# MayDomine/Burst-Attention

Measured on NVIDIA H100. Metric: attention fwd+bwd TFLOPS/s (bs=1, H=32, d=128, bf16; seq in config, default 262144 on N > 1 GPUs, 65536 on one), aggregate over GPUs, higher is better.
Workload: dtype bf16

## Files before the change

### burst-attention_b200/csrc/fwd_sm90.cuh

```cuda
#pragma once
#include <math.h>
#include <stdlib.h>

#include "doc_sm90.cuh"
#include "host_common.h"
#include "sm90_ptx.cuh"

namespace ba {

constexpr int kBlockM = 128;
constexpr int kBlockN = 128;
constexpr int kKStages = 2;
constexpr int kVStages = 2;
constexpr int kBoxBytes = 128 * 64 * 2;
constexpr int kFwdThreads = 384;

struct FwdParams {
  float* o_acc;
  int64_t oacc_sb, oacc_ss, oacc_sh;
  float* lse;
  int64_t lse_sb, lse_sh;
  void* o_out;
  int64_t oout_sb, oout_ss, oout_sh;
  int B, Sq, Sk, H;
  int G;
  float scale_log2;
  const float* bias;
  int64_t bias_sb, bias_sh;
  int causal;
  int causal_off;
  int load_state;
  int store_lowp;
  int lo;
  const float* slopes;
  int64_t slopes_sb;
  int64_t dist0;
  int pstride;
  const int* cu;
  int n_docs;
  int q_pos0, k_pos0;
};

struct __align__(8) FwdBarriers {
  uint64_t q_full;
  uint64_t k_full[kKStages], k_empty[kKStages];
  uint64_t b_full[kKStages];
  uint64_t v_full[kVStages], v_empty[kVStages];
};

template <int kD>
struct FwdLayout {
  static_assert(kD == 64 || kD == 128, "head dim 64 or 128");
  static constexpr uint32_t kTileB = 128 * kD * 2;
  static constexpr int kBoxes = kD / 64;
  static constexpr uint32_t kOffQ = 0;
  static constexpr uint32_t kOffK = kTileB;
  static constexpr uint32_t kOffV = kOffK + kKStages * kTileB;
  static constexpr uint32_t kOffBias = kOffV + kVStages * kTileB;
  static constexpr uint32_t kOffBars = kOffBias + kKStages * kBlockN * 4;
  static constexpr int kSmemBytes = kOffBars + 256 ;
  static_assert(kSmemBytes <= 232448, "forward kernel exceeds 227 KiB of shared memory");
};

__device__ __forceinline__ int fwd_trip_count(int r0, const FwdParams& p) {
  if (r0 >= p.Sq) return 0;
  int r_last = min(r0 + 63, p.Sq - 1);
  int max_limit = p.causal ? min(r_last + p.causal_off, p.Sk - 1) : p.Sk - 1;
  return max_limit < 0 ? 0 : max_limit / kBlockN + 1;
}

__device__ __forceinline__ int fwd_first_tile(int r0, const FwdParams& p) { return max(0, r0 + p.lo) / kBlockN; }

__device__ __forceinline__ void fwd_doc_range(int r0, const FwdParams& p, int* first, int* end) {
  *first = *end = 0;
  if (r0 >= p.Sq) return;
  const int r_last = min(r0 + 63, p.Sq - 1);
  int k_lo, k_hi, unused;
  doc_interval(p.q_pos0 + p.pstride * r0, p.cu, p.n_docs, p.k_pos0, p.pstride, p.Sk, &k_lo, &unused);
  doc_interval(p.q_pos0 + p.pstride * r_last, p.cu, p.n_docs, p.k_pos0, p.pstride, p.Sk, &unused, &k_hi);
  const int f = max(fwd_first_tile(r0, p), k_lo / kBlockN);
  const int e = min(fwd_trip_count(r0, p), (k_hi + kBlockN - 1) / kBlockN);
  if (e > f) *first = f, *end = e;
}

__device__ __forceinline__ int64_t alibi_dref(int a, const FwdParams& p) {
  const int64_t hi = (int64_t)p.pstride * a + p.dist0, lo = hi - (int64_t)p.pstride * (p.Sk - 1);
  return max((int64_t)0, max(lo, -hi));
}

__device__ __forceinline__ int64_t alibi_carried_ref(int64_t dref, float m0, float slope2) {
  if (slope2 > 0.f) {
    const float cap = fmaxf(0.f, -m0) / slope2;
    if (cap < (float)dref) return (int64_t)cap;
  }
  return dref;
}

template <bool kBF16, int kD, bool kBias, bool kBand, bool kAlibi, bool kDoc = false>
__device__ __forceinline__ void fwd_chunk_body(const CUtensorMap& tmQ, const CUtensorMap& tmK, const CUtensorMap& tmV,
                                               const FwdParams& p) {
  static_assert(!(kBias && kAlibi), "ALiBi is not combined with the key bias");
  static_assert(!kDoc || (kBand && !kBias && !kAlibi), "documents run on the band path, without key bias or ALiBi");
  extern __shared__ __align__(1024) uint8_t smem_raw[];
  uint8_t* smem = smem_raw;
  if ((smem_u32(smem) & 1023u) != 0) __trap();
  using L = FwdLayout<kD>;
  constexpr uint32_t kTileBytes = L::kTileB;
  constexpr int kBoxes = L::kBoxes, kOReg = kD / 2;
  uint8_t* sQ = smem + L::kOffQ;
  uint8_t* sK = smem + L::kOffK;
  uint8_t* sV = smem + L::kOffV;
  float* sBias = reinterpret_cast<float*>(smem + L::kOffBias);
  FwdBarriers* bars = reinterpret_cast<FwdBarriers*>(smem + L::kOffBars);

  const int warp = __shfl_sync(0xffffffffu, threadIdx.x >> 5, 0);
  const int lane = threadIdx.x & 31;
  const int h = blockIdx.y, b = blockIdx.z;
  const int row0 = (p.causal ? (int)(gridDim.x - 1 - blockIdx.x) : (int)blockIdx.x) * kBlockM;
  int n_tiles = max(fwd_trip_count(row0, p), fwd_trip_count(row0 + 64, p));
  int t0 = 0;
  if constexpr (kBand) {
    t0 = min(fwd_first_tile(row0, p), n_tiles);
    n_tiles -= t0;
  }
  if constexpr (kDoc) {
    int f0, e0, f1, e1;
    fwd_doc_range(row0, p, &f0, &e0);
    fwd_doc_range(row0 + 64, p, &f1, &e1);
    t0 = e0 > f0 ? (e1 > f1 ? min(f0, f1) : f0) : f1;
    n_tiles = max(0, max(e0, e1) - t0);
  }

  if (threadIdx.x == 0) {
    tma_prefetch_desc(&tmQ);
    tma_prefetch_desc(&tmK);
    tma_prefetch_desc(&tmV);
    mbar_init(&bars->q_full, 1);
    for (int i = 0; i < kKStages; ++i) {
      mbar_init(&bars->k_full[i], 1);
      mbar_init(&bars->k_empty[i], 8);
      mbar_init(&bars->b_full[i], 1);
    }
    for (int i = 0; i < kVStages; ++i) {
      mbar_init(&bars->v_full[i], 1);
      mbar_init(&bars->v_empty[i], 8);
    }
    fence_mbar_init();
  }
  __syncthreads();

  if (warp < 4) {
    reg_alloc_dec<40>();
    if (warp != 0) return;
    const int hk = h / p.G;
    if (lane == 0) {
      mbar_arrive_expect_tx(&bars->q_full, kTileBytes);
      for (int half = 0; half < kBoxes; ++half)
        tma_load_4d(sQ + half * kBoxBytes, &tmQ, &bars->q_full, half * 64, h, row0, b);
    }
    for (int i = 0; i < n_tiles; ++i) {
      const int ks = i % kKStages, kph = (i / kKStages) & 1;
      mbar_wait(&bars->k_empty[ks], kph ^ 1);
      if (lane == 0) {
        mbar_arrive_expect_tx(&bars->k_full[ks], kTileBytes);
        for (int half = 0; half < kBoxes; ++half)
          tma_load_4d(sK + ks * kTileBytes + half * kBoxBytes, &tmK, &bars->k_full[ks], half * 64, hk,
                      (t0 + i) * kBlockN, b);
      }
      if constexpr (kBias) {
#pragma unroll
        for (int j = 0; j < 4; ++j) {
          const int key = (t0 + i) * kBlockN + lane + 32 * j;
          float x = 0.f;
          if (key < p.Sk) x = __ldg(p.bias + (int64_t)b * p.bias_sb + (int64_t)h * p.bias_sh + key) * kLog2e;
          sBias[ks * kBlockN + lane + 32 * j] = x;
        }
        __syncwarp();
        if (lane == 0) mbar_arrive(&bars->b_full[ks]);
      }
      if (lane == 0) {
        const int vs = i % kVStages, vph = (i / kVStages) & 1;
        mbar_wait(&bars->v_empty[vs], vph ^ 1);
        mbar_arrive_expect_tx(&bars->v_full[vs], kTileBytes);
        for (int half = 0; half < kBoxes; ++half)
          tma_load_4d(sV + vs * kTileBytes + half * kBoxBytes, &tmV, &bars->v_full[vs], half * 64, hk,
                      (t0 + i) * kBlockN, b);
      }
      __syncwarp();
    }
    return;
  }

  reg_alloc_inc<232>();
  const int wg = (threadIdx.x >> 7) - 1;
  const int w = warp & 3, g = lane >> 2, t = lane & 3;
  const int r_lo = row0 + wg * 64 + 16 * w + g;
  const int rows[2] = {r_lo, r_lo + 8};
  [[maybe_unused]] int doc_first = 0, doc_end = 0, doc_lo[2] = {0, 0}, doc_hi[2] = {0, 0};
  if constexpr (kDoc) {
    fwd_doc_range(row0 + wg * 64, p, &doc_first, &doc_end);
#pragma unroll
    for (int r = 0; r < 2; ++r)
      if (rows[r] < p.Sq)
        doc_interval(p.q_pos0 + p.pstride * rows[r], p.cu, p.n_docs, p.k_pos0, p.pstride, p.Sk, &doc_lo[r], &doc_hi[r]);
  }
  const int n_mine = kDoc ? doc_end : fwd_trip_count(row0 + wg * 64, p);
  const float scale_log2 = p.scale_log2;
  int limit[2];
#pragma unroll
  for (int r = 0; r < 2; ++r) limit[r] = p.causal ? min(rows[r] + p.causal_off, p.Sk - 1) : p.Sk - 1;
  if constexpr (kDoc) {
#pragma unroll
    for (int r = 0; r < 2; ++r) limit[r] = min(limit[r], doc_hi[r] - 1);
  }
  const int limit_min = min(limit[0], limit[1]);
  int my0 = 0, lo_limit[2] = {0, 0};
  if constexpr (kBand) {
    my0 = fwd_first_tile(row0 + wg * 64, p);
    lo_limit[0] = rows[0] + p.lo;
    lo_limit[1] = rows[1] + p.lo;
  }
  if constexpr (kDoc) {
    my0 = doc_first;
#pragma unroll
    for (int r = 0; r < 2; ++r) lo_limit[r] = max(lo_limit[r], doc_lo[r]);
  }
  const int lo_limit_max = max(lo_limit[0], lo_limit[1]);
  float slope2 = 0.f;
  int64_t dref[2] = {0, 0};
  if constexpr (kAlibi) {
    slope2 = __ldg(p.slopes + (int64_t)b * p.slopes_sb + h) * kLog2e;
    dref[0] = alibi_dref(rows[0], p);
    dref[1] = alibi_dref(rows[1], p);
  }

  float o[kOReg];
  float m[2] = {-INFINITY, -INFINITY}, l[2] = {0.f, 0.f};
#pragma unroll
  for (int i = 0; i < kOReg; ++i) o[i] = 0.f;
  if (p.load_state) {
#pragma unroll
    for (int r = 0; r < 2; ++r) {
      if (rows[r] >= p.Sq) continue;
      const float lse_prev = p.lse[(int64_t)b * p.lse_sb + (int64_t)h * p.lse_sh + rows[r]];
      if (lse_prev != -INFINITY) {
        m[r] = lse_prev * kLog2e;
        if constexpr (kAlibi) {
          dref[r] = alibi_carried_ref(dref[r], m[r], slope2);
          m[r] += slope2 * (float)dref[r];
        }
        l[r] = t == 0 ? 1.f : 0.f;
      }
      const float* src = p.o_acc + (int64_t)b * p.oacc_sb + (int64_t)rows[r] * p.oacc_ss + (int64_t)h * p.oacc_sh;
#pragma unroll
      for (int c = 0; c < kD / 8; ++c) {
        const float2 f = __ldg(reinterpret_cast<const float2*>(src + 8 * c + 2 * t));
        o[4 * c + 2 * r] = f.x;
        o[4 * c + 2 * r + 1] = f.y;
      }
    }
  }

  const uint32_t q_base = smem_u32(sQ) + wg * 64 * 128;
  mbar_wait(&bars->q_full, 0);
  for (int i = 0; i < n_tiles; ++i) {
    const int ks = i % kKStages, kph = (i / kKStages) & 1;
    const int vs = i % kVStages, vph = (i / kVStages) & 1;
    const bool work = kBand ? (t0 + i >= my0 && t0 + i < n_mine) : i < n_mine;
    mbar_wait(&bars->k_full[ks], kph);
    float sc[64];
    if (work) {
      const uint32_t k_base = smem_u32(sK + ks * kTileBytes);
      wgmma_fence();
#pragma unroll
      for (int kk = 0; kk < kD / 16; ++kk) {
        const uint32_t off = (kk >> 2) * kBoxBytes + (kk & 3) * 32;
        wgmma_ss_n128<kBF16, 0, 0>(sc, make_desc(q_base + off, 16, 1024), make_desc(k_base + off, 16, 1024),
                                   kk > 0 ? 1u : 0u);
      }
      wgmma_commit();
      wgmma_wait<0>();
      fence_regs<64>(sc);
      const int key0 = (t0 + i) * kBlockN;
      if constexpr (kBias) {
        mbar_wait(&bars->b_full[ks], kph);
        const float* bias = sBias + ks * kBlockN;
#pragma unroll
        for (int c = 0; c < 16; ++c) {
          const float2 bb = *reinterpret_cast<const float2*>(bias + 8 * c + 2 * t);
#pragma unroll
          for (int r = 0; r < 2; ++r) {
            sc[4 * c + 2 * r] = fmaf(sc[4 * c + 2 * r], scale_log2, bb.x);
            sc[4 * c + 2 * r + 1] = fmaf(sc[4 * c + 2 * r + 1], scale_log2, bb.y);
          }
        }
      } else if constexpr (kAlibi) {
        const int64_t base = (int64_t)p.pstride * (row0 + wg * 64 - key0) + p.dist0;
        const int64_t dmin = base - (int64_t)p.pstride * (kBlockN - 1), dmax = base + (int64_t)p.pstride * 63;
        const float pf = (float)p.pstride;
        if (dmin >= 0 || dmax <= 0) {
          const int sg = dmin >= 0 ? 1 : -1;
          float rowb[2];
#pragma unroll
          for (int r = 0; r < 2; ++r)
            rowb[r] = -slope2 * (float)(sg * ((int64_t)p.pstride * (rows[r] - key0) + p.dist0) - dref[r]);
          const float ks = sg > 0 ? slope2 * pf : -slope2 * pf, kt = ks * (float)(2 * t);
#pragma unroll
          for (int c = 0; c < 16; ++c)
#pragma unroll
            for (int e = 0; e < 4; ++e)
              sc[4 * c + e] = fmaf(sc[4 * c + e], scale_log2, rowb[e >> 1] + fmaf(ks, (float)(8 * c + (e & 1)), kt));
        } else {
          float dr[2], dreff[2];
#pragma unroll
          for (int r = 0; r < 2; ++r) {
            dr[r] = (float)((int64_t)p.pstride * (rows[r] - key0 - 2 * t) + p.dist0);
            dreff[r] = slope2 * (float)dref[r];
          }
#pragma unroll
          for (int c = 0; c < 16; ++c)
#pragma unroll
            for (int e = 0; e < 4; ++e)
              sc[4 * c + e] = fmaf(-slope2, fabsf(fmaf(-pf, (float)(8 * c + (e & 1)), dr[e >> 1])),
                                   fmaf(sc[4 * c + e], scale_log2, dreff[e >> 1]));
        }
      } else {
#pragma unroll
        for (int j = 0; j < 64; ++j) sc[j] *= scale_log2;
      }
      if (key0 + kBlockN - 1 > limit_min) {
#pragma unroll
        for (int c = 0; c < 16; ++c)
#pragma unroll
          for (int e = 0; e < 4; ++e)
            if (key0 + 8 * c + 2 * t + (e & 1) > limit[e >> 1]) sc[4 * c + e] = -INFINITY;
      }
      if constexpr (kBand) {
        if (key0 < lo_limit_max) {
#pragma unroll
          for (int c = 0; c < 16; ++c)
#pragma unroll
            for (int e = 0; e < 4; ++e)
              if (key0 + 8 * c + 2 * t + (e & 1) < lo_limit[e >> 1]) sc[4 * c + e] = -INFINITY;
        }
      }
    }
    __syncwarp();
    if (lane == 0) mbar_arrive(&bars->k_empty[ks]);
    if (work) {
      uint32_t pa[32];
#pragma unroll
      for (int r = 0; r < 2; ++r) {
        float mx = -INFINITY;
#pragma unroll
        for (int c = 0; c < 16; ++c) mx = fmaxf(mx, fmaxf(sc[4 * c + 2 * r], sc[4 * c + 2 * r + 1]));
        mx = fmaxf(mx, __shfl_xor_sync(0xffffffffu, mx, 1));
        mx = fmaxf(mx, __shfl_xor_sync(0xffffffffu, mx, 2));
        const float m_new = fmaxf(m[r], mx);
        const float f = (m[r] == -INFINITY) ? 0.f : ex2(m[r] - m_new);
        const float neg_m = (m_new == -INFINITY) ? 0.f : -m_new;
        m[r] = m_new;
        float sum = 0.f;
#pragma unroll
        for (int c = 0; c < 16; ++c) {
          const float p0 = ex2(sc[4 * c + 2 * r] + neg_m), p1 = ex2(sc[4 * c + 2 * r + 1] + neg_m);
          sc[4 * c + 2 * r] = p0;
          sc[4 * c + 2 * r + 1] = p1;
          sum += p0 + p1;
        }
        l[r] = l[r] * f + sum;
#pragma unroll
        for (int c = 0; c < kD / 8; ++c) {
          o[4 * c + 2 * r] *= f;
          o[4 * c + 2 * r + 1] *= f;
        }
      }
#pragma unroll
      for (int j = 0; j < 32; ++j) pa[j] = pack2<kBF16>(sc[2 * j], sc[2 * j + 1]);
      mbar_wait(&bars->v_full[vs], vph);
      const uint32_t v_base = smem_u32(sV + vs * kTileBytes);
      fence_regs<32>(pa);
      fence_regs<kOReg>(o);
      wgmma_fence();
#pragma unroll
      for (int kk = 0; kk < kBlockN / 16; ++kk) {
        const uint64_t dv = make_desc(v_base + kk * 16 * 128, kBoxBytes, 1024);
        if constexpr (kD == 128) wgmma_rs_n128<kBF16, 1>(o, pa + 4 * kk, dv, 1u);
        else wgmma_rs_n64<kBF16, 1>(o, pa + 4 * kk, dv, 1u);
      }
      wgmma_commit();
      wgmma_wait<0>();
      fence_regs<kOReg>(o);
    } else {
      mbar_wait(&bars->v_full[vs], vph);
    }
    __syncwarp();
    if (lane == 0) mbar_arrive(&bars->v_empty[vs]);
  }

#pragma unroll
  for (int r = 0; r < 2; ++r) {
    float lr = l[r];
    lr += __shfl_xor_sync(0xffffffffu, lr, 1);
    lr += __shfl_xor_sync(0xffffffffu, lr, 2);
    const int row = rows[r];
    if (row >= p.Sq) continue;
    const float inv_l = lr > 0.f ? 1.f / lr : 0.f;
    if constexpr (kAlibi) {
      if (t == 0)
        p.lse[(int64_t)b * p.lse_sb + (int64_t)h * p.lse_sh + row] =
            lr > 0.f ? (m[r] + lg2(lr) - slope2 * (float)dref[r]) * kLn2 : -INFINITY;
    } else {
      if (t == 0) p.lse[(int64_t)b * p.lse_sb + (int64_t)h * p.lse_sh + row] = lr > 0.f ? (m[r] + lg2(lr)) * kLn2 : -INFINITY;
    }
    if (p.store_lowp) {
      uint16_t* dst = reinterpret_cast<uint16_t*>(p.o_out) + (int64_t)b * p.oout_sb + (int64_t)row * p.oout_ss +
                      (int64_t)h * p.oout_sh + 2 * t;
#pragma unroll
      for (int c = 0; c < kD / 8; ++c)
        *reinterpret_cast<uint32_t*>(dst + 8 * c) = pack2<kBF16>(o[4 * c + 2 * r] * inv_l, o[4 * c + 2 * r + 1] * inv_l);
    } else {
      float* dst = p.o_acc + (int64_t)b * p.oacc_sb + (int64_t)row * p.oacc_ss + (int64_t)h * p.oacc_sh + 2 * t;
#pragma unroll
      for (int c = 0; c < kD / 8; ++c)
        *reinterpret_cast<float2*>(dst + 8 * c) = make_float2(o[4 * c + 2 * r] * inv_l, o[4 * c + 2 * r + 1] * inv_l);
    }
  }
}

template <bool kBF16, int kD, bool kBias, bool kBand>
__global__ void __launch_bounds__(kFwdThreads, 1)
fwd_chunk_kernel(const __grid_constant__ CUtensorMap tmQ, const __grid_constant__ CUtensorMap tmK,
                 const __grid_constant__ CUtensorMap tmV, const FwdParams p) {
  fwd_chunk_body<kBF16, kD, kBias, kBand, false>(tmQ, tmK, tmV, p);
}

template <bool kBF16, int kD, bool kBand>
__global__ void __launch_bounds__(kFwdThreads, 1)
fwd_alibi_kernel(const __grid_constant__ CUtensorMap tmQ, const __grid_constant__ CUtensorMap tmK,
                 const __grid_constant__ CUtensorMap tmV, const FwdParams p) {
  fwd_chunk_body<kBF16, kD, false, kBand, true>(tmQ, tmK, tmV, p);
}

template <bool kBF16, int kD>
__global__ void __launch_bounds__(kFwdThreads, 1)
fwd_doc_kernel(const __grid_constant__ CUtensorMap tmQ, const __grid_constant__ CUtensorMap tmK,
               const __grid_constant__ CUtensorMap tmV, const FwdParams p) {
  fwd_chunk_body<kBF16, kD, false, true, false, true>(tmQ, tmK, tmV, p);
}

template <bool kBand>
inline int launch_fwd(int dtype, int D, bool bias, const CUtensorMap& tmQ, const CUtensorMap& tmK,
                      const CUtensorMap& tmV, const FwdParams& p, cudaStream_t stream) {
  const bool bf16 = dtype == BA_DTYPE_BF16;
  void (*kern)(CUtensorMap, CUtensorMap, CUtensorMap, FwdParams);
  if (bias)
    kern = D == 64 ? (bf16 ? fwd_chunk_kernel<true, 64, true, kBand> : fwd_chunk_kernel<false, 64, true, kBand>)
                   : (bf16 ? fwd_chunk_kernel<true, 128, true, kBand> : fwd_chunk_kernel<false, 128, true, kBand>);
  else
    kern = D == 64 ? (bf16 ? fwd_chunk_kernel<true, 64, false, kBand> : fwd_chunk_kernel<false, 64, false, kBand>)
                   : (bf16 ? fwd_chunk_kernel<true, 128, false, kBand> : fwd_chunk_kernel<false, 128, false, kBand>);
  const int smem = D == 64 ? FwdLayout<64>::kSmemBytes : FwdLayout<128>::kSmemBytes;
  BA_CHECK_CUDA(cudaFuncSetAttribute(kern, cudaFuncAttributeMaxDynamicSharedMemorySize, smem));
  dim3 grid((p.Sq + kBlockM - 1) / kBlockM, p.H, p.B);
  kern<<<grid, kFwdThreads, smem, stream>>>(tmQ, tmK, tmV, p);
  BA_CHECK_CUDA(cudaGetLastError());
  return BA_OK;
}

int launch_fwd_band(int dtype, int D, bool bias, const CUtensorMap& tmQ, const CUtensorMap& tmK,
                    const CUtensorMap& tmV, const FwdParams& p, cudaStream_t stream);
int launch_fwd_alibi(int dtype, int D, bool band, const CUtensorMap& tmQ, const CUtensorMap& tmK,
                     const CUtensorMap& tmV, const FwdParams& p, cudaStream_t stream);
int launch_fwd_doc(int dtype, int D, const CUtensorMap& tmQ, const CUtensorMap& tmK, const CUtensorMap& tmV,
                   const FwdParams& p, cudaStream_t stream);

}
```

Before: 503.2.

## Overlap QK^T of next tile with PV of previous tile in forward consumer

Restructures the consumer warpgroup loop into a software pipeline. The S=QK^T wgmma for tile i is issued together with the P·V wgmma for tile i-1, so softmax of tile i runs while the PV matmul is in flight. Skipped tiles outside the work range are now handled by separate pre and post loops that only cycle the barriers. This costs extra live registers, since sc, pa and o are all held at once, which risks spills and also changes the K/V release ordering.

```diff
diff --git a/burst-attention_b200/csrc/fwd_sm90.cuh b/burst-attention_b200/csrc/fwd_sm90.cuh
--- a/burst-attention_b200/csrc/fwd_sm90.cuh
+++ b/burst-attention_b200/csrc/fwd_sm90.cuh
@@ -262,141 +262,187 @@
   }
 
   const uint32_t q_base = smem_u32(sQ) + wg * 64 * 128;
+  int s_begin = 0, s_end = n_mine;
+  if constexpr (kBand) s_begin = max(my0 - t0, 0), s_end = n_mine - t0;
+  s_begin = min(s_begin, n_tiles);
+  s_end = max(min(s_end, n_tiles), s_begin);
+
+  const auto wait_k = [&](int i) { mbar_wait(&bars->k_full[i % kKStages], (i / kKStages) & 1); };
+  const auto wait_v = [&](int i) { mbar_wait(&bars->v_full[i % kVStages], (i / kVStages) & 1); };
+  const auto release_k = [&](int i) {
+    __syncwarp();
+    if (lane == 0) mbar_arrive(&bars->k_empty[i % kKStages]);
+  };
+  const auto release_v = [&](int i) {
+    __syncwarp();
+    if (lane == 0) mbar_arrive(&bars->v_empty[i % kVStages]);
+  };
+  const auto skip = [&](int i) {
+    wait_k(i);
+    release_k(i);
+    wait_v(i);
+    release_v(i);
+  };
+  const auto issue_s = [&](int i, float* sc) {
+    const uint32_t k_base = smem_u32(sK + (i % kKStages) * kTileBytes);
+    wgmma_fence();
+#pragma unroll
+    for (int kk = 0; kk < kD / 16; ++kk) {
+      const uint32_t off = (kk >> 2) * kBoxBytes + (kk & 3) * 32;
+      wgmma_ss_n128<kBF16, 0, 0>(sc, make_desc(q_base + off, 16, 1024), make_desc(k_base + off, 16, 1024),
+                                 kk > 0 ? 1u : 0u);
+    }
+    wgmma_commit();
+  };
+  const auto issue_pv = [&](int i, uint32_t* pa) {
+    wait_v(i);
+    const uint32_t v_base = smem_u32(sV + (i % kVStages) * kTileBytes);
+    fence_regs<32>(pa);
+    fence_regs<kOReg>(o);
+    wgmma_fence();
+#pragma unroll
+    for (int kk = 0; kk < kBlockN / 16; ++kk) {
+      const uint64_t dv = make_desc(v_base + kk * 16 * 128, kBoxBytes, 1024);
+      if constexpr (kD == 128) wgmma_rs_n128<kBF16, 1>(o, pa + 4 * kk, dv, 1u);
+      else wgmma_rs_n64<kBF16, 1>(o, pa + 4 * kk, dv, 1u);
+    }
+    wgmma_commit();
+  };
+  const auto scores = [&](int i, float* sc) {
+    const int key0 = (t0 + i) * kBlockN;
+    if constexpr (kBias) {
+      const int ks = i % kKStages;
+      mbar_wait(&bars->b_full[ks], (i / kKStages) & 1);
+      const float* bias = sBias + ks * kBlockN;
+#pragma unroll
+      for (int c = 0; c < 16; ++c) {
+        const float2 bb = *reinterpret_cast<const float2*>(bias + 8 * c + 2 * t);
+#pragma unroll
+        for (int r = 0; r < 2; ++r) {
+          sc[4 * c + 2 * r] = fmaf(sc[4 * c + 2 * r], scale_log2, bb.x);
+          sc[4 * c + 2 * r + 1] = fmaf(sc[4 * c + 2 * r + 1], scale_log2, bb.y);
+        }
+      }
+    } else if constexpr (kAlibi) {
+      const int64_t base = (int64_t)p.pstride * (row0 + wg * 64 - key0) + p.dist0;
+      const int64_t dmin = base - (int64_t)p.pstride * (kBlockN - 1), dmax = base + (int64_t)p.pstride * 63;
+      const float pf = (float)p.pstride;
+      if (dmin >= 0 || dmax <= 0) {
+        const int sg = dmin >= 0 ? 1 : -1;
+        float rowb[2];
+#pragma unroll
+        for (int r = 0; r < 2; ++r)
+          rowb[r] = -slope2 * (float)(sg * ((int64_t)p.pstride * (rows[r] - key0) + p.dist0) - dref[r]);
+        const float ks = sg > 0 ? slope2 * pf : -slope2 * pf, kt = ks * (float)(2 * t);
+#pragma unroll
+        for (int c = 0; c < 16; ++c)
+#pragma unroll
+          for (int e = 0; e < 4; ++e)
+            sc[4 * c + e] = fmaf(sc[4 * c + e], scale_log2, rowb[e >> 1] + fmaf(ks, (float)(8 * c + (e & 1)), kt));
+      } else {
+        float dr[2], dreff[2];
+#pragma unroll
+        for (int r = 0; r < 2; ++r) {
+          dr[r] = (float)((int64_t)p.pstride * (rows[r] - key0 - 2 * t) + p.dist0);
+          dreff[r] = slope2 * (float)dref[r];
+        }
+#pragma unroll
+        for (int c = 0; c < 16; ++c)
+#pragma unroll
+          for (int e = 0; e < 4; ++e)
+            sc[4 * c + e] = fmaf(-slope2, fabsf(fmaf(-pf, (float)(8 * c + (e & 1)), dr[e >> 1])),
+                                 fmaf(sc[4 * c + e], scale_log2, dreff[e >> 1]));
+      }
+    } else {
+#pragma unroll
+      for (int j = 0; j < 64; ++j) sc[j] *= scale_log2;
+    }
+    if (key0 + kBlockN - 1 > limit_min) {
+#pragma unroll
+      for (int c = 0; c < 16; ++c)
+#pragma unroll
+        for (int e = 0; e < 4; ++e)
+          if (key0 + 8 * c + 2 * t + (e & 1) > limit[e >> 1]) sc[4 * c + e] = -INFINITY;
+    }
+    if constexpr (kBand) {
+      if (key0 < lo_limit_max) {
+#pragma unroll
+        for (int c = 0; c < 16; ++c)
+#pragma unroll
+          for (int e = 0; e < 4; ++e)
+            if (key0 + 8 * c + 2 * t + (e & 1) < lo_limit[e >> 1]) sc[4 * c + e] = -INFINITY;
+      }
+    }
+    release_k(i);
+  };
+  const auto softmax = [&](float* sc, float* f) {
+#pragma unroll
+    for (int r = 0; r < 2; ++r) {
+      float mx = -INFINITY;
+#pragma unroll
+      for (int c = 0; c < 16; ++c) mx = fmaxf(mx, fmaxf(sc[4 * c + 2 * r], sc[4 * c + 2 * r + 1]));
+      mx = fmaxf(mx, __shfl_xor_sync(0xffffffffu, mx, 1));
+      mx = fmaxf(mx, __shfl_xor_sync(0xffffffffu, mx, 2));
+      const float m_new = fmaxf(m[r], mx);
+      f[r] = (m[r] == -INFINITY) ? 0.f : ex2(m[r] - m_new);
+      const float neg_m = (m_new == -INFINITY) ? 0.f : -m_new;
+      m[r] = m_new;
+      float sum = 0.f;
+#pragma unroll
+      for (int c = 0; c < 16; ++c) {
+        const float p0 = ex2(sc[4 * c + 2 * r] + neg_m), p1 = ex2(sc[4 * c + 2 * r + 1] + neg_m);
+        sc[4 * c + 2 * r] = p0;
+        sc[4 * c + 2 * r + 1] = p1;
+        sum += p0 + p1;
+      }
+      l[r] = l[r] * f[r] + sum;
+    }
+  };
+  const auto rescale_pack = [&](const float* sc, const float* f, uint32_t* pa) {
+#pragma unroll
+    for (int r = 0; r < 2; ++r)
+#pragma unroll
+      for (int c = 0; c < kD / 8; ++c) {
+        o[4 * c + 2 * r] *= f[r];
+        o[4 * c + 2 * r + 1] *= f[r];
+      }
+#pragma unroll
+    for (int j = 0; j < 32; ++j) pa[j] = pack2<kBF16>(sc[2 * j], sc[2 * j + 1]);
+  };
+
   mbar_wait(&bars->q_full, 0);
-  for (int i = 0; i < n_tiles; ++i) {
-    const int ks = i % kKStages, kph = (i / kKStages) & 1;
-    const int vs = i % kVStages, vph = (i / kVStages) & 1;
-    const bool work = kBand ? (t0 + i >= my0 && t0 + i < n_mine) : i < n_mine;
-    mbar_wait(&bars->k_full[ks], kph);
-    float sc[64];
-    if (work) {
-      const uint32_t k_base = smem_u32(sK + ks * kTileBytes);
-      wgmma_fence();
-#pragma unroll
-      for (int kk = 0; kk < kD / 16; ++kk) {
-        const uint32_t off = (kk >> 2) * kBoxBytes + (kk & 3) * 32;
-        wgmma_ss_n128<kBF16, 0, 0>(sc, make_desc(q_base + off, 16, 1024), make_desc(k_base + off, 16, 1024),
-                                   kk > 0 ? 1u : 0u);
-      }
-      wgmma_commit();
-      wgmma_wait<0>();
+  for (int i = 0; i < s_begin; ++i) skip(i);
+  if (s_end > s_begin) {
+    float sc[64], f[2];
+    uint32_t pa[32];
+    wait_k(s_begin);
+    issue_s(s_begin, sc);
+    wgmma_wait<0>();
+    fence_regs<64>(sc);
+    scores(s_begin, sc);
+    softmax(sc, f);
+    rescale_pack(sc, f, pa);
+    if (s_begin + 1 < s_end) wait_k(s_begin + 1);
+    for (int i = s_begin + 1; i < s_end; ++i) {
+      issue_s(i, sc);
+      issue_pv(i - 1, pa);
+      wgmma_wait<1>();
       fence_regs<64>(sc);
-      const int key0 = (t0 + i) * kBlockN;
-      if constexpr (kBias) {
-        mbar_wait(&bars->b_full[ks], kph);
-        const float* bias = sBias + ks * kBlockN;
-#pragma unroll
-        for (int c = 0; c < 16; ++c) {
-          const float2 bb = *reinterpret_cast<const float2*>(bias + 8 * c + 2 * t);
-#pragma unroll
-          for (int r = 0; r < 2; ++r) {
-            sc[4 * c + 2 * r] = fmaf(sc[4 * c + 2 * r], scale_log2, bb.x);
-            sc[4 * c + 2 * r + 1] = fmaf(sc[4 * c + 2 * r + 1], scale_log2, bb.y);
-          }
-        }
-      } else if constexpr (kAlibi) {
-        const int64_t base = (int64_t)p.pstride * (row0 + wg * 64 - key0) + p.dist0;
-        const int64_t dmin = base - (int64_t)p.pstride * (kBlockN - 1), dmax = base + (int64_t)p.pstride * 63;
-        const float pf = (float)p.pstride;
-        if (dmin >= 0 || dmax <= 0) {
-          const int sg = dmin >= 0 ? 1 : -1;
-          float rowb[2];
-#pragma unroll
-          for (int r = 0; r < 2; ++r)
-            rowb[r] = -slope2 * (float)(sg * ((int64_t)p.pstride * (rows[r] - key0) + p.dist0) - dref[r]);
-          const float ks = sg > 0 ? slope2 * pf : -slope2 * pf, kt = ks * (float)(2 * t);
-#pragma unroll
-          for (int c = 0; c < 16; ++c)
-#pragma unroll
-            for (int e = 0; e < 4; ++e)
-              sc[4 * c + e] = fmaf(sc[4 * c + e], scale_log2, rowb[e >> 1] + fmaf(ks, (float)(8 * c + (e & 1)), kt));
-        } else {
-          float dr[2], dreff[2];
-#pragma unroll
-          for (int r = 0; r < 2; ++r) {
-            dr[r] = (float)((int64_t)p.pstride * (rows[r] - key0 - 2 * t) + p.dist0);
-            dreff[r] = slope2 * (float)dref[r];
-          }
-#pragma unroll
-          for (int c = 0; c < 16; ++c)
-#pragma unroll
-            for (int e = 0; e < 4; ++e)
-              sc[4 * c + e] = fmaf(-slope2, fabsf(fmaf(-pf, (float)(8 * c + (e & 1)), dr[e >> 1])),
-                                   fmaf(sc[4 * c + e], scale_log2, dreff[e >> 1]));
-        }
-      } else {
-#pragma unroll
-        for (int j = 0; j < 64; ++j) sc[j] *= scale_log2;
-      }
-      if (key0 + kBlockN - 1 > limit_min) {
-#pragma unroll
-        for (int c = 0; c < 16; ++c)
-#pragma unroll
-          for (int e = 0; e < 4; ++e)
-            if (key0 + 8 * c + 2 * t + (e & 1) > limit[e >> 1]) sc[4 * c + e] = -INFINITY;
-      }
-      if constexpr (kBand) {
-        if (key0 < lo_limit_max) {
-#pragma unroll
-          for (int c = 0; c < 16; ++c)
-#pragma unroll
-            for (int e = 0; e < 4; ++e)
-              if (key0 + 8 * c + 2 * t + (e & 1) < lo_limit[e >> 1]) sc[4 * c + e] = -INFINITY;
-        }
-      }
-    }
-    __syncwarp();
-    if (lane == 0) mbar_arrive(&bars->k_empty[ks]);
-    if (work) {
-      uint32_t pa[32];
-#pragma unroll
-      for (int r = 0; r < 2; ++r) {
-        float mx = -INFINITY;
-#pragma unroll
-        for (int c = 0; c < 16; ++c) mx = fmaxf(mx, fmaxf(sc[4 * c + 2 * r], sc[4 * c + 2 * r + 1]));
-        mx = fmaxf(mx, __shfl_xor_sync(0xffffffffu, mx, 1));
-        mx = fmaxf(mx, __shfl_xor_sync(0xffffffffu, mx, 2));
-        const float m_new = fmaxf(m[r], mx);
-        const float f = (m[r] == -INFINITY) ? 0.f : ex2(m[r] - m_new);
-        const float neg_m = (m_new == -INFINITY) ? 0.f : -m_new;
-        m[r] = m_new;
-        float sum = 0.f;
-#pragma unroll
-        for (int c = 0; c < 16; ++c) {
-          const float p0 = ex2(sc[4 * c + 2 * r] + neg_m), p1 = ex2(sc[4 * c + 2 * r + 1] + neg_m);
-          sc[4 * c + 2 * r] = p0;
-          sc[4 * c + 2 * r + 1] = p1;
-          sum += p0 + p1;
-        }
-        l[r] = l[r] * f + sum;
-#pragma unroll
-        for (int c = 0; c < kD / 8; ++c) {
-          o[4 * c + 2 * r] *= f;
-          o[4 * c + 2 * r + 1] *= f;
-        }
-      }
-#pragma unroll
-      for (int j = 0; j < 32; ++j) pa[j] = pack2<kBF16>(sc[2 * j], sc[2 * j + 1]);
-      mbar_wait(&bars->v_full[vs], vph);
-      const uint32_t v_base = smem_u32(sV + vs * kTileBytes);
-      fence_regs<32>(pa);
-      fence_regs<kOReg>(o);
-      wgmma_fence();
-#pragma unroll
-      for (int kk = 0; kk < kBlockN / 16; ++kk) {
-        const uint64_t dv = make_desc(v_base + kk * 16 * 128, kBoxBytes, 1024);
-        if constexpr (kD == 128) wgmma_rs_n128<kBF16, 1>(o, pa + 4 * kk, dv, 1u);
-        else wgmma_rs_n64<kBF16, 1>(o, pa + 4 * kk, dv, 1u);
-      }
-      wgmma_commit();
+      scores(i, sc);
+      softmax(sc, f);
+      if (i + 1 < s_end) wait_k(i + 1);
       wgmma_wait<0>();
       fence_regs<kOReg>(o);
-    } else {
-      mbar_wait(&bars->v_full[vs], vph);
-    }
-    __syncwarp();
-    if (lane == 0) mbar_arrive(&bars->v_empty[vs]);
-  }
+      fence_regs<32>(pa);
+      release_v(i - 1);
+      rescale_pack(sc, f, pa);
+    }
+    issue_pv(s_end - 1, pa);
+    wgmma_wait<0>();
+    fence_regs<kOReg>(o);
+    release_v(s_end - 1);
+  }
+  for (int i = s_end; i < n_tiles; ++i) skip(i);
 
 #pragma unroll
   for (int r = 0; r < 2; ++r) {
```

New measurement: 506.4, median of 6. Within noise of the previous version (+0.6%).

## Software-pipeline forward loop to overlap P·V wgmma with next tile's softmax

Applied to the files above, without the earlier changes.

Restructures the forward consumer loop so that after issuing QK^T for tile i, the PV wgmma for tile i-1 is issued asynchronously and runs while softmax for tile i is computed. Skipped tiles before and after the active range are handled by separate loops that only cycle the barriers, which removes the per-iteration work branch. The O rescale is deferred until after the previous PV completes. This raises register pressure because sc, pa and o are all live at once, and it reorders barrier releases.

```diff
diff --git a/burst-attention_b200/csrc/fwd_sm90.cuh b/burst-attention_b200/csrc/fwd_sm90.cuh
--- a/burst-attention_b200/csrc/fwd_sm90.cuh
+++ b/burst-attention_b200/csrc/fwd_sm90.cuh
@@ -261,142 +261,175 @@
     }
   }
 
+  const int ia = min(max(my0 - t0, 0), n_tiles);
+  const int ie = min(max(n_mine - t0, ia), n_tiles);
   const uint32_t q_base = smem_u32(sQ) + wg * 64 * 128;
+  auto release = [&](uint64_t* bar) {
+    __syncwarp();
+    if (lane == 0) mbar_arrive(bar);
+  };
+  auto skip = [&](int i) {
+    mbar_wait(&bars->k_full[i % kKStages], (i / kKStages) & 1);
+    release(&bars->k_empty[i % kKStages]);
+    mbar_wait(&bars->v_full[i % kVStages], (i / kVStages) & 1);
+    release(&bars->v_empty[i % kVStages]);
+  };
+  float sc[64];
+  uint32_t pa[32];
+  auto issue_s = [&](int i) {
+    const int ks = i % kKStages;
+    mbar_wait(&bars->k_full[ks], (i / kKStages) & 1);
+    const uint32_t k_base = smem_u32(sK + ks * kTileBytes);
+    fence_regs<64>(sc);
+    wgmma_fence();
+#pragma unroll
+    for (int kk = 0; kk < kD / 16; ++kk) {
+      const uint32_t off = (kk >> 2) * kBoxBytes + (kk & 3) * 32;
+      wgmma_ss_n128<kBF16, 0, 0>(sc, make_desc(q_base + off, 16, 1024), make_desc(k_base + off, 16, 1024),
+                                 kk > 0 ? 1u : 0u);
+    }
+    wgmma_commit();
+  };
+  auto issue_pv = [&](int i) {
+    const int vs = i % kVStages;
+    mbar_wait(&bars->v_full[vs], (i / kVStages) & 1);
+    const uint32_t v_base = smem_u32(sV + vs * kTileBytes);
+    fence_regs<32>(pa);
+    fence_regs<kOReg>(o);
+    wgmma_fence();
+#pragma unroll
+    for (int kk = 0; kk < kBlockN / 16; ++kk) {
+      const uint64_t dv = make_desc(v_base + kk * 16 * 128, kBoxBytes, 1024);
+      if constexpr (kD == 128) wgmma_rs_n128<kBF16, 1>(o, pa + 4 * kk, dv, 1u);
+      else wgmma_rs_n64<kBF16, 1>(o, pa + 4 * kk, dv, 1u);
+    }
+    wgmma_commit();
+  };
+  auto softmax = [&](int i, float* f) {
+    fence_regs<64>(sc);
+    const int ks = i % kKStages;
+    const int key0 = (t0 + i) * kBlockN;
+    if constexpr (kBias) {
+      mbar_wait(&bars->b_full[ks], (i / kKStages) & 1);
+      const float* bias = sBias + ks * kBlockN;
+#pragma unroll
+      for (int c = 0; c < 16; ++c) {
+        const float2 bb = *reinterpret_cast<const float2*>(bias + 8 * c + 2 * t);
+#pragma unroll
+        for (int r = 0; r < 2; ++r) {
+          sc[4 * c + 2 * r] = fmaf(sc[4 * c + 2 * r], scale_log2, bb.x);
+          sc[4 * c + 2 * r + 1] = fmaf(sc[4 * c + 2 * r + 1], scale_log2, bb.y);
+        }
+      }
+    } else if constexpr (kAlibi) {
+      const int64_t base = (int64_t)p.pstride * (row0 + wg * 64 - key0) + p.dist0;
+      const int64_t dmin = base - (int64_t)p.pstride * (kBlockN - 1), dmax = base + (int64_t)p.pstride * 63;
+      const float pf = (float)p.pstride;
+      if (dmin >= 0 || dmax <= 0) {
+        const int sg = dmin >= 0 ? 1 : -1;
+        float rowb[2];
+#pragma unroll
+        for (int r = 0; r < 2; ++r)
+          rowb[r] = -slope2 * (float)(sg * ((int64_t)p.pstride * (rows[r] - key0) + p.dist0) - dref[r]);
+        const float ks = sg > 0 ? slope2 * pf : -slope2 * pf, kt = ks * (float)(2 * t);
+#pragma unroll
+        for (int c = 0; c < 16; ++c)
+#pragma unroll
+          for (int e = 0; e < 4; ++e)
+            sc[4 * c + e] = fmaf(sc[4 * c + e], scale_log2, rowb[e >> 1] + fmaf(ks, (float)(8 * c + (e & 1)), kt));
+      } else {
+        float dr[2], dreff[2];
+#pragma unroll
+        for (int r = 0; r < 2; ++r) {
+          dr[r] = (float)((int64_t)p.pstride * (rows[r] - key0 - 2 * t) + p.dist0);
+          dreff[r] = slope2 * (float)dref[r];
+        }
+#pragma unroll
+        for (int c = 0; c < 16; ++c)
+#pragma unroll
+          for (int e = 0; e < 4; ++e)
+            sc[4 * c + e] = fmaf(-slope2, fabsf(fmaf(-pf, (float)(8 * c + (e & 1)), dr[e >> 1])),
+                                 fmaf(sc[4 * c + e], scale_log2, dreff[e >> 1]));
+      }
+    } else {
+#pragma unroll
+      for (int j = 0; j < 64; ++j) sc[j] *= scale_log2;
+    }
+    if (key0 + kBlockN - 1 > limit_min) {
+#pragma unroll
+      for (int c = 0; c < 16; ++c)
+#pragma unroll
+        for (int e = 0; e < 4; ++e)
+          if (key0 + 8 * c + 2 * t + (e & 1) > limit[e >> 1]) sc[4 * c + e] = -INFINITY;
+    }
+    if constexpr (kBand) {
+      if (key0 < lo_limit_max) {
+#pragma unroll
+        for (int c = 0; c < 16; ++c)
+#pragma unroll
+          for (int e = 0; e < 4; ++e)
+            if (key0 + 8 * c + 2 * t + (e & 1) < lo_limit[e >> 1]) sc[4 * c + e] = -INFINITY;
+      }
+    }
+    release(&bars->k_empty[ks]);
+#pragma unroll
+    for (int r = 0; r < 2; ++r) {
+      float mx = -INFINITY;
+#pragma unroll
+      for (int c = 0; c < 16; ++c) mx = fmaxf(mx, fmaxf(sc[4 * c + 2 * r], sc[4 * c + 2 * r + 1]));
+      mx = fmaxf(mx, __shfl_xor_sync(0xffffffffu, mx, 1));
+      mx = fmaxf(mx, __shfl_xor_sync(0xffffffffu, mx, 2));
+      const float m_new = fmaxf(m[r], mx);
+      f[r] = (m[r] == -INFINITY) ? 0.f : ex2(m[r] - m_new);
+      const float neg_m = (m_new == -INFINITY) ? 0.f : -m_new;
+      m[r] = m_new;
+      float sum = 0.f;
+#pragma unroll
+      for (int c = 0; c < 16; ++c) {
+        const float p0 = ex2(sc[4 * c + 2 * r] + neg_m), p1 = ex2(sc[4 * c + 2 * r + 1] + neg_m);
+        sc[4 * c + 2 * r] = p0;
+        sc[4 * c + 2 * r + 1] = p1;
+        sum += p0 + p1;
+      }
+      l[r] = l[r] * f[r] + sum;
+    }
+  };
+  auto rescale_pack = [&](const float* f) {
+#pragma unroll
+    for (int c = 0; c < kD / 8; ++c)
+#pragma unroll
+      for (int e = 0; e < 4; ++e) o[4 * c + e] *= f[e >> 1];
+#pragma unroll
+    for (int j = 0; j < 32; ++j) pa[j] = pack2<kBF16>(sc[2 * j], sc[2 * j + 1]);
+  };
+
   mbar_wait(&bars->q_full, 0);
-  for (int i = 0; i < n_tiles; ++i) {
-    const int ks = i % kKStages, kph = (i / kKStages) & 1;
-    const int vs = i % kVStages, vph = (i / kVStages) & 1;
-    const bool work = kBand ? (t0 + i >= my0 && t0 + i < n_mine) : i < n_mine;
-    mbar_wait(&bars->k_full[ks], kph);
-    float sc[64];
-    if (work) {
-      const uint32_t k_base = smem_u32(sK + ks * kTileBytes);
-      wgmma_fence();
-#pragma unroll
-      for (int kk = 0; kk < kD / 16; ++kk) {
-        const uint32_t off = (kk >> 2) * kBoxBytes + (kk & 3) * 32;
-        wgmma_ss_n128<kBF16, 0, 0>(sc, make_desc(q_base + off, 16, 1024), make_desc(k_base + off, 16, 1024),
-                                   kk > 0 ? 1u : 0u);
-      }
-      wgmma_commit();
+  for (int i = 0; i < ia; ++i) skip(i);
+  if (ia < ie) {
+    float f[2];
+    issue_s(ia);
+    wgmma_wait<0>();
+    softmax(ia, f);
+    rescale_pack(f);
+    for (int i = ia + 1; i < ie; ++i) {
+      issue_s(i);
       wgmma_wait<0>();
-      fence_regs<64>(sc);
-      const int key0 = (t0 + i) * kBlockN;
-      if constexpr (kBias) {
-        mbar_wait(&bars->b_full[ks], kph);
-        const float* bias = sBias + ks * kBlockN;
-#pragma unroll
-        for (int c = 0; c < 16; ++c) {
-          const float2 bb = *reinterpret_cast<const float2*>(bias + 8 * c + 2 * t);
-#pragma unroll
-          for (int r = 0; r < 2; ++r) {
-            sc[4 * c + 2 * r] = fmaf(sc[4 * c + 2 * r], scale_log2, bb.x);
-            sc[4 * c + 2 * r + 1] = fmaf(sc[4 * c + 2 * r + 1], scale_log2, bb.y);
-          }
-        }
-      } else if constexpr (kAlibi) {
-        const int64_t base = (int64_t)p.pstride * (row0 + wg * 64 - key0) + p.dist0;
-        const int64_t dmin = base - (int64_t)p.pstride * (kBlockN - 1), dmax = base + (int64_t)p.pstride * 63;
-        const float pf = (float)p.pstride;
-        if (dmin >= 0 || dmax <= 0) {
-          const int sg = dmin >= 0 ? 1 : -1;
-          float rowb[2];
-#pragma unroll
-          for (int r = 0; r < 2; ++r)
-            rowb[r] = -slope2 * (float)(sg * ((int64_t)p.pstride * (rows[r] - key0) + p.dist0) - dref[r]);
-          const float ks = sg > 0 ? slope2 * pf : -slope2 * pf, kt = ks * (float)(2 * t);
-#pragma unroll
-          for (int c = 0; c < 16; ++c)
-#pragma unroll
-            for (int e = 0; e < 4; ++e)
-              sc[4 * c + e] = fmaf(sc[4 * c + e], scale_log2, rowb[e >> 1] + fmaf(ks, (float)(8 * c + (e & 1)), kt));
-        } else {
-          float dr[2], dreff[2];
-#pragma unroll
-          for (int r = 0; r < 2; ++r) {
-            dr[r] = (float)((int64_t)p.pstride * (rows[r] - key0 - 2 * t) + p.dist0);
-            dreff[r] = slope2 * (float)dref[r];
-          }
-#pragma unroll
-          for (int c = 0; c < 16; ++c)
-#pragma unroll
-            for (int e = 0; e < 4; ++e)
-              sc[4 * c + e] = fmaf(-slope2, fabsf(fmaf(-pf, (float)(8 * c + (e & 1)), dr[e >> 1])),
-                                   fmaf(sc[4 * c + e], scale_log2, dreff[e >> 1]));
-        }
-      } else {
-#pragma unroll
-        for (int j = 0; j < 64; ++j) sc[j] *= scale_log2;
-      }
-      if (key0 + kBlockN - 1 > limit_min) {
-#pragma unroll
-        for (int c = 0; c < 16; ++c)
-#pragma unroll
-          for (int e = 0; e < 4; ++e)
-            if (key0 + 8 * c + 2 * t + (e & 1) > limit[e >> 1]) sc[4 * c + e] = -INFINITY;
-      }
-      if constexpr (kBand) {
-        if (key0 < lo_limit_max) {
-#pragma unroll
-          for (int c = 0; c < 16; ++c)
-#pragma unroll
-            for (int e = 0; e < 4; ++e)
-              if (key0 + 8 * c + 2 * t + (e & 1) < lo_limit[e >> 1]) sc[4 * c + e] = -INFINITY;
-        }
-      }
-    }
-    __syncwarp();
-    if (lane == 0) mbar_arrive(&bars->k_empty[ks]);
-    if (work) {
-      uint32_t pa[32];
-#pragma unroll
-      for (int r = 0; r < 2; ++r) {
-        float mx = -INFINITY;
-#pragma unroll
-        for (int c = 0; c < 16; ++c) mx = fmaxf(mx, fmaxf(sc[4 * c + 2 * r], sc[4 * c + 2 * r + 1]));
-        mx = fmaxf(mx, __shfl_xor_sync(0xffffffffu, mx, 1));
-        mx = fmaxf(mx, __shfl_xor_sync(0xffffffffu, mx, 2));
-        const float m_new = fmaxf(m[r], mx);
-        const float f = (m[r] == -INFINITY) ? 0.f : ex2(m[r] - m_new);
-        const float neg_m = (m_new == -INFINITY) ? 0.f : -m_new;
-        m[r] = m_new;
-        float sum = 0.f;
-#pragma unroll
-        for (int c = 0; c < 16; ++c) {
-          const float p0 = ex2(sc[4 * c + 2 * r] + neg_m), p1 = ex2(sc[4 * c + 2 * r + 1] + neg_m);
-          sc[4 * c + 2 * r] = p0;
-          sc[4 * c + 2 * r + 1] = p1;
-          sum += p0 + p1;
-        }
-        l[r] = l[r] * f + sum;
-#pragma unroll
-        for (int c = 0; c < kD / 8; ++c) {
-          o[4 * c + 2 * r] *= f;
-          o[4 * c + 2 * r + 1] *= f;
-        }
-      }
-#pragma unroll
-      for (int j = 0; j < 32; ++j) pa[j] = pack2<kBF16>(sc[2 * j], sc[2 * j + 1]);
-      mbar_wait(&bars->v_full[vs], vph);
-      const uint32_t v_base = smem_u32(sV + vs * kTileBytes);
-      fence_regs<32>(pa);
-      fence_regs<kOReg>(o);
-      wgmma_fence();
-#pragma unroll
-      for (int kk = 0; kk < kBlockN / 16; ++kk) {
-        const uint64_t dv = make_desc(v_base + kk * 16 * 128, kBoxBytes, 1024);
-        if constexpr (kD == 128) wgmma_rs_n128<kBF16, 1>(o, pa + 4 * kk, dv, 1u);
-        else wgmma_rs_n64<kBF16, 1>(o, pa + 4 * kk, dv, 1u);
-      }
-      wgmma_commit();
+      issue_pv(i - 1);
+      softmax(i, f);
+      if (i + 1 < ie) mbar_wait(&bars->k_full[(i + 1) % kKStages], ((i + 1) / kKStages) & 1);
       wgmma_wait<0>();
       fence_regs<kOReg>(o);
-    } else {
-      mbar_wait(&bars->v_full[vs], vph);
-    }
-    __syncwarp();
-    if (lane == 0) mbar_arrive(&bars->v_empty[vs]);
-  }
+      fence_regs<32>(pa);
+      release(&bars->v_empty[(i - 1) % kVStages]);
+      rescale_pack(f);
+    }
+    issue_pv(ie - 1);
+    wgmma_wait<0>();
+    fence_regs<kOReg>(o);
+    fence_regs<32>(pa);
+    release(&bars->v_empty[(ie - 1) % kVStages]);
+  }
+  for (int i = ie; i < n_tiles; ++i) skip(i);
 
 #pragma unroll
   for (int r = 0; r < 2; ++r) {
```

Measured after the change: 505.3 before, 507.9 after, median of 6. Within noise of the previous version (+0.5%).
